# flysnowtiger/GRL

Measured on AMD Instinct MI355X. Metric: clip-features/sec, higher is better.
Workload: dtype f32; 1 GPU; GRL eval clip features (ResNet-50 s1 trunk + GCE + TRL + Siamese attention -> 6144-d), BASELINE configs[1]; clips_per_gpu=32, seq_len=4, frame=256x128, parallelism=replicas x1 (no collective), math=f32

## Files before the change

grl_amd/csrc/gemm_f32.hip:

```cpp
#include <type_traits>
#include <hip/hip_runtime.h>
#include <stdint.h>
#include <stdio.h>
#include <stdlib.h>
#include "../../include/grl_hip.h"
#include "common.h"

namespace {

constexpr int BK = 32;
#ifndef GRL_GEMM_KO
#define GRL_GEMM_KO 0
#endif
constexpr int SEG_STAGES = 16;
#ifndef GRL_GEMM_RING3
#define GRL_GEMM_RING3 1
#endif
#ifndef GRL_GEMM_PIPE
#define GRL_GEMM_PIPE 1
#endif

#ifndef GRL_GEMM_EV_OCC3
#define GRL_GEMM_EV_OCC3 1
#endif

typedef __attribute__((address_space(3))) char* lds_cptr_t;
#pragma clang diagnostic push
#pragma clang diagnostic ignored "-Winline-asm"
__device__ __forceinline__ void dma16_hidden(const char* sbase, uint32_t voff, uint32_t lds) {
    asm volatile("s_mov_b32 m0, %2\n\ts_nop 0\n\tglobal_load_lds_dwordx4 %0, %1" ::"v"(voff), "s"(sbase), "s"(lds) : "memory", "m0");
}
__device__ __forceinline__ void dma16_hidden_v(const char* vaddr, uint32_t lds) {
    asm volatile("s_mov_b32 m0, %1\n\ts_nop 0\n\tglobal_load_lds_dwordx4 %0, off" ::"v"(vaddr), "s"(lds) : "memory", "m0");
}
#pragma clang diagnostic pop

__device__ uint4 g_zero_chunks[8];

struct RowInfo {
    int64_t base;
    int iy0, ix0;
};

constexpr int EV_NONE = 0, EV_AFFINE = 1, EV_SQDIFF = 2;
template <int BM, int BN, bool CONV, int MATH, bool SEG, bool DMA = false, bool SPLITK = false, int EV = EV_NONE>
__global__ __launch_bounds__(256, (GRL_GEMM_EV_OCC3 && EV != EV_NONE && BN == 64) ? 3 : 2) void gemm_f32_kernel(const GrlGemm p_in, const int tiles_n,
                                                                                               const int num_tiles, const int vec_epi_in) {
    static_assert(EV == EV_NONE || (MATH == 0 && BM == 128 && DMA && !SEG && !SPLITK && GRL_GEMM_PIPE), "eval variants: the hand-scheduled fp32 kernels");
    static_assert(EV != EV_SQDIFF || (BN == 128 && !CONV), "SQDIFF: dense, 128 x 128");
    const int vec_epi = EV == EV_NONE ? vec_epi_in : EV == EV_SQDIFF ? (vec_epi_in & 8) | 1 : vec_epi_in & 9;
    GrlGemm p_seg;
    if constexpr (SPLITK) {
        p_seg = p_in;
        const int seg = blockIdx.y, kseg = SEG_STAGES * BK;
        p_seg.a = p_in.a + (int64_t)seg * kseg;
        p_seg.w = p_in.w + (int64_t)seg * kseg;
        p_seg.K = min(kseg, p_in.K - seg * kseg);
        p_seg.y = p_in.splitk_ws + (int64_t)seg * p_in.M * p_in.N;
        p_seg.ldy = p_in.N;
        p_seg.scale = p_seg.shift = p_seg.res = p_seg.gbias = p_seg.rowscale = nullptr;
        p_seg.stats = nullptr;
        p_seg.relu = 0;
    }
    GrlGemm p_ev;
    if constexpr (EV != EV_NONE) {
        p_ev = p_in;
        p_ev.epilogue = EV == EV_SQDIFF ? GRL_EPI_SQDIFF : GRL_EPI_AFFINE;
        p_ev.stats = nullptr;
        p_ev.rowscale = p_ev.rnorm = p_ev.cnorm = nullptr;
        p_ev.bn_z = p_ev.bn_mean = p_ev.bn_invstd = p_ev.bn_mscale = p_ev.bn_mbeta = nullptr;
        p_ev.bn_bits = nullptr;
        p_ev.splitk_ws = nullptr;
        p_ev.kblock = 0;
        p_ev.out_f32 = 0;
        if constexpr (EV == EV_SQDIFF) { p_ev.gbias = nullptr; p_ev.relu = 0; }
    }
    const GrlGemm& p = SPLITK ? p_seg : EV != EV_NONE ? p_ev : p_in;
    constexpr int WTM = BM / 2, WTN = BN / 2;
    constexpr int MT = WTM / 32, NT = WTN / 32;
    constexpr int ESZ = MATH == 2 ? 2 : 4;
    constexpr int EPC = 16 / ESZ;
    constexpr int KST = 8 * EPC;
    auto gp = [](const float* base, int64_t elem_off) {
        return reinterpret_cast<const f32x4*>(reinterpret_cast<const char*>(base) + elem_off * ESZ);
    };
    constexpr int A_ITEMS = BM / 32, B_ITEMS = BN / 32;
    constexpr bool RING = GRL_GEMM_PIPE && GRL_GEMM_RING3 && DMA && MATH == 2 && BM == 128 && BN == 64;
    constexpr int NST = RING ? 3 : 2;
    constexpr bool PIPE = (GRL_GEMM_PIPE && DMA && MATH == 0 && BM == 128) || RING;
    extern __shared__ __attribute__((aligned(16))) float smem[];
    float* As = smem;
    float* Bs = smem + NST * BM * BK;
    constexpr int PL = MATH == 3 ? 2 : 1;
    char* const Ah = reinterpret_cast<char*>(smem);
    char* const Bh = Ah + 2 * PL * BM * 64;

    const int tid = threadIdx.x, lane = tid & 63, wave = PIPE ? __builtin_amdgcn_readfirstlane(tid >> 6) : tid >> 6;
    const int wm = wave >> 1, wn = wave & 1;
    const int ld_row = tid >> 3, ld_chunk = tid & 7;
    const int d_row = lane >> 3, d_chunk = lane & 7;

    RowInfo ai[A_ITEMS];
    int64_t bofs[B_ITEMS];
    const char* dma_a[DMA ? BM / 32 : 1];
    const char* dma_b[DMA ? BN / 32 : 1];
    int dma_iy0[DMA && CONV ? BM / 32 : 1], dma_ix0[DMA && CONV ? BM / 32 : 1];
    const char* cbase[PIPE && CONV ? BM / 32 : 1];
    uint32_t cmask[PIPE && CONV ? BM / 32 : 1];
    uint32_t pv_a[PIPE ? BM / 32 : 1], pv_b[PIPE ? BN / 32 : 1];
    const char *pbase_a = nullptr, *pbase_b = nullptr;
    int m0, n0, tile_m;
    const int tiles_m = num_tiles / tiles_n;
    const int panel_w = (vec_epi & 8) && tiles_n > 8 && (tiles_n & 7) == 0 ? 8 : 0;
    auto setup_tile = [&](int t) {
        int bid = t;
        {
            const int q = num_tiles >> 3, r = num_tiles & 7, xcd = bid & 7;
            bid = (xcd < r ? xcd * (q + 1) : r * (q + 1) + (xcd - r) * q) + (bid >> 3);
        }
        int tile_n;
        if (panel_w > 0) {
            const int per_panel = tiles_m * panel_w;
            const int pn = bid / per_panel, rem = bid - pn * per_panel;
            tile_m = rem / panel_w;
            tile_n = pn * panel_w + (rem - tile_m * panel_w);
        } else {
            tile_m = bid / tiles_n;
            tile_n = bid - tile_m * tiles_n;
        }
        m0 = tile_m * BM;
        n0 = tile_n * BN;
#pragma unroll
        for (int i = 0; i < A_ITEMS; ++i) {
            int m = m0 + ld_row + 32 * i;
            m = m < p.M ? m : p.M - 1;
            if (CONV) {
                const int hw = p.Ho * p.Wo;
                const int img = m / hw, rem = m - img * hw;
                const int oy = rem / p.Wo, ox = rem - oy * p.Wo;
                ai[i].base = (int64_t)img * p.H * p.W * p.C;
                ai[i].iy0 = oy * p.stride - p.pad;
                ai[i].ix0 = ox * p.stride - p.pad;
            } else {
                ai[i].base = (int64_t)m * p.lda;
                ai[i].iy0 = ai[i].ix0 = 0;
            }
        }
#pragma unroll
        for (int i = 0; i < B_ITEMS; ++i) {
            int n = n0 + ld_row + 32 * i;
            n = n < p.N ? n : p.N - 1;
            bofs[i] = (int64_t)n * p.ldw;
        }
        if constexpr (PIPE) {
            pbase_b = reinterpret_cast<const char*>(p.w) + ((int64_t)n0 * p.ldw) * ESZ;
#pragma unroll
            for (int i = 0; i < BN / 32; ++i) {
                const int r = (wave + 4 * i) * 8 + d_row;
                const int n = n0 + r < p.N ? r : p.N - 1 - n0;
                pv_b[i] = (uint32_t)(n * p.ldw * ESZ + ((d_chunk ^ ((r >> 1) & 7)) << 4));
            }
        }
        if constexpr (PIPE && !CONV) {
            pbase_a = reinterpret_cast<const char*>(p.a) + ((int64_t)m0 * p.lda) * ESZ;
#pragma unroll
            for (int i = 0; i < BM / 32; ++i) {
                const int r = (wave + 4 * i) * 8 + d_row;
                const int m = m0 + r < p.M ? r : p.M - 1 - m0;
                pv_a[i] = (uint32_t)(m * p.lda * ESZ + ((d_chunk ^ ((r >> 1) & 7)) << 4));
            }
        } else if constexpr (DMA) {
#pragma unroll
            for (int i = 0; i < BM / 32; ++i) {
                const int r = (wave + 4 * i) * 8 + d_row;
                int m = m0 + r;
                m = m < p.M ? m : p.M - 1;
                if constexpr (CONV) {
                    const int hw = p.Ho * p.Wo;
                    const int img = m / hw, rem = m - img * hw;
                    const int oy = rem / p.Wo, ox = rem - oy * p.Wo;
                    dma_a[i] = reinterpret_cast<const char*>(p.a) + ((int64_t)img * p.H * p.W * p.C) * ESZ + ((d_chunk ^ ((r >> 1) & 7)) << 4);
                    dma_iy0[i] = oy * p.stride - p.pad;
                    dma_ix0[i] = ox * p.stride - p.pad;
                    if constexpr (PIPE) {
                        cbase[i] = dma_a[i] + ((int64_t)(dma_iy0[i] * p.W + dma_ix0[i]) * p.C) * ESZ;
                        uint32_t mk = 0;
                        for (int ky = 0, t = 0; ky < p.kh; ++ky)
                            for (int kx = 0; kx < p.kw; ++kx, ++t)
                                if ((unsigned)(dma_iy0[i] + ky) < (unsigned)p.H && (unsigned)(dma_ix0[i] + kx) < (unsigned)p.W) mk |= 1u << t;
                        cmask[i] = mk;
                    }
                } else {
                    dma_a[i] = reinterpret_cast<const char*>(p.a) + ((int64_t)m * p.lda) * ESZ + ((d_chunk ^ ((r >> 1) & 7)) << 4);
                }
            }
#pragma unroll
            for (int i = 0; i < BN / 32; ++i) {
                const int r = (wave + 4 * i) * 8 + d_row;
                int n = n0 + r;
                n = n < p.N ? n : p.N - 1;
                dma_b[i] = reinterpret_cast<const char*>(p.w) + ((int64_t)n * p.ldw) * ESZ + ((d_chunk ^ ((r >> 1) & 7)) << 4);
            }
        }
    };

    const uint32_t lds_base = (uint32_t)(size_t)((lds_cptr_t) reinterpret_cast<char*>(smem));
    int pky = 0, pkx = 0, pc0 = 0;
    const char* pn_src[PIPE && CONV ? BM / 32 : 1];
    const char* czero = reinterpret_cast<const char*>(g_zero_chunks) + (d_chunk << 4);
    if constexpr (PIPE && CONV) asm volatile("" : "+v"(czero));
    auto conv_tap_reset = [&]() { pky = pkx = pc0 = 0; };
    auto conv_tap_advance = [&]() {
        pc0 += KST;
        if (pc0 >= p.C) {
            pc0 = 0;
            if (++pkx == p.kw) { pkx = 0; ++pky; }
        }
    };
    auto conv_addrs = [&]() {
        if constexpr (PIPE && CONV) {
            const int64_t toff = ((int64_t)(pky * p.W + pkx) * p.C + pc0) * ESZ;
            const uint32_t bit = 1u << (pky * p.kw + pkx);
#pragma unroll
            for (int i = 0; i < BM / 32; ++i)
                pn_src[i] = (cmask[i] & bit) ? cbase[i] + toff : czero;
        }
    };
    auto dma_piece = [&](int buf, int ks, int i) {
        if constexpr (PIPE) {
            const int64_t kb = (int64_t)ks * KST * ESZ;
            if (i < BM / 32) {
                const uint32_t dst = lds_base + (uint32_t)((buf * BM * BK) * 4 + (wave + 4 * i) * 1024);
                if constexpr (CONV) dma16_hidden_v(pn_src[i], dst);
                else dma16_hidden(pbase_a + kb, pv_a[i], dst);
            } else
                dma16_hidden(pbase_b + kb, pv_b[i - BM / 32],
                             lds_base + (uint32_t)((NST * BM * BK + buf * BN * BK) * 4 + (wave + 4 * (i - BM / 32)) * 1024));
        }
    };
    auto dma_stage = [&](int buf, int ks) {
        if constexpr (PIPE) {
            if constexpr (CONV) { conv_tap_reset(); conv_addrs(); }
#pragma unroll
            for (int i = 0; i < BM / 32 + BN / 32; ++i) dma_piece(buf, ks, i);
        } else if constexpr (DMA) {
            if (GRL_GEMM_KO & 8) ks = 0;
            char* const Asb = reinterpret_cast<char*>(As + buf * BM * BK);
            char* const Bsb = reinterpret_cast<char*>(Bs + buf * BN * BK);
            const int64_t kb = (int64_t)ks * KST * ESZ;
            if constexpr (CONV) {
                const int k0 = ks * KST;
                const int tap = k0 / p.C, c0 = k0 - tap * p.C;
                const int ky = tap / p.kw, kx = tap - ky * p.kw;
                const char* const zsrc = reinterpret_cast<const char*>(g_zero_chunks) + (d_chunk << 4);
#pragma unroll
                for (int i = 0; i < BM / 32; ++i) {
                    const int rb = wave + 4 * i;
                    const int iy = dma_iy0[i] + ky, ix = dma_ix0[i] + kx;
                    const bool ok = (unsigned)iy < (unsigned)p.H && (unsigned)ix < (unsigned)p.W;
                    const char* src = ok ? dma_a[i] + ((int64_t)(iy * p.W + ix) * p.C + c0) * ESZ : zsrc;
                    __builtin_amdgcn_global_load_lds((const __attribute__((address_space(1))) void*)src,
                                                     (__attribute__((address_space(3))) void*)(Asb + rb * 1024), 16, 0, 0);
                }
            } else {
#pragma unroll
            for (int i = 0; i < BM / 32; ++i) {
                const int rb = wave + 4 * i;
                __builtin_amdgcn_global_load_lds((const __attribute__((address_space(1))) void*)(dma_a[i] + kb),
                                                 (__attribute__((address_space(3))) void*)(Asb + rb * 1024), 16, 0, 0);
            }
            }
#pragma unroll
            for (int i = 0; i < BN / 32; ++i) {
                const int rb = wave + 4 * i;
                __builtin_amdgcn_global_load_lds((const __attribute__((address_space(1))) void*)(dma_b[i] + kb),
                                                 (__attribute__((address_space(3))) void*)(Bsb + rb * 1024), 16, 0, 0);
            }
        }
    };

    f32x4 areg[A_ITEMS], breg[B_ITEMS];
    auto load_stage = [&](int ks) {
        if constexpr (DMA) return;
        const int k0 = ks * KST;
        if (CONV) {
            const int tap = k0 / p.C, c0 = k0 - tap * p.C;
            const int ky = tap / p.kw, kx = tap - ky * p.kw;
#pragma unroll
            for (int i = 0; i < A_ITEMS; ++i) {
                const int iy = ai[i].iy0 + ky, ix = ai[i].ix0 + kx;
                const bool ok = (unsigned)iy < (unsigned)p.H && (unsigned)ix < (unsigned)p.W;
                const int64_t pix = ok ? (int64_t)iy * p.W + ix : 0;
                f32x4 v = *gp(p.a, ai[i].base + pix * p.C + c0 + ld_chunk * EPC);
#pragma unroll
                for (int e = 0; e < 4; ++e) v[e] = ok ? v[e] : 0.f;
                areg[i] = v;
            }
        } else {
#pragma unroll
            for (int i = 0; i < A_ITEMS; ++i)
                areg[i] = *gp(p.a, ai[i].base + k0 + ld_chunk * EPC);
        }
#pragma unroll
        for (int i = 0; i < B_ITEMS; ++i)
            breg[i] = *gp(p.w, bofs[i] + k0 + ld_chunk * EPC);
    };
    auto split_store = [&](char* plane0, int plane_bytes, int row, const f32x4 v) {
        const int off = row * 64 + (((ld_chunk >> 1) ^ ((row >> 2) & 3)) << 4) + (ld_chunk & 1) * 8;
        bf16x4 hi;
#pragma unroll
        for (int e = 0; e < 4; ++e) hi[e] = (__bf16)v[e];
        *reinterpret_cast<bf16x4*>(plane0 + off) = hi;
        if (MATH == 3) {
            bf16x4 lo;
#pragma unroll
            for (int e = 0; e < 4; ++e) lo[e] = (__bf16)(v[e] - (float)hi[e]);
            *reinterpret_cast<bf16x4*>(plane0 + plane_bytes + off) = lo;
        }
    };
    auto store_stage = [&](int buf) {
        if constexpr (DMA) return;
        if constexpr (MATH == 0 || MATH == 2) {
#pragma unroll
            for (int i = 0; i < A_ITEMS; ++i) {
                const int row = ld_row + 32 * i;
                *reinterpret_cast<f32x4*>(As + buf * BM * BK + row * BK +
                                          ((ld_chunk ^ ((row >> 1) & 7)) << 2)) = areg[i];
            }
#pragma unroll
            for (int i = 0; i < B_ITEMS; ++i) {
                const int row = ld_row + 32 * i;
                *reinterpret_cast<f32x4*>(Bs + buf * BN * BK + row * BK +
                                          ((ld_chunk ^ ((row >> 1) & 7)) << 2)) = breg[i];
            }
        } else {
#pragma unroll
            for (int i = 0; i < A_ITEMS; ++i)
                split_store(Ah + buf * PL * BM * 64, BM * 64, ld_row + 32 * i, areg[i]);
#pragma unroll
            for (int i = 0; i < B_ITEMS; ++i)
                split_store(Bh + buf * PL * BN * 64, BN * 64, ld_row + 32 * i, breg[i]);
        }
    };

    const int nk = p.K / KST;
    const int frow = lane & 31, fhalf = lane >> 5;
    const int col_l = lane & 31;

    int t = blockIdx.x;
    setup_tile(t);
    load_stage(0);
    dma_stage(0, 0);
    for (;;) {
    f32x16 acc[MT][NT], tot[SEG ? MT : 1][SEG ? NT : 1];
#pragma unroll
    for (int i = 0; i < MT; ++i)
#pragma unroll
        for (int j = 0; j < NT; ++j)
#pragma unroll
            for (int r = 0; r < 16; ++r) acc[i][j][r] = 0.f;
    if constexpr (SEG) {
#pragma unroll
        for (int i = 0; i < MT; ++i)
#pragma unroll
            for (int j = 0; j < NT; ++j)
#pragma unroll
                for (int r = 0; r < 16; ++r) tot[i][j][r] = 0.f;
    }

    store_stage(0);
    constexpr int NP_ALL = BM / 32 + BN / 32;
    if constexpr (RING) {
        if (nk > 1) {
            if constexpr (CONV) { conv_tap_advance(); conv_addrs(); }
#pragma unroll
            for (int i = 0; i < NP_ALL; ++i) dma_piece(1, 1, i);
            asm volatile("s_waitcnt vmcnt(%0)" ::"n"(NP_ALL) : "memory");
        } else {
            asm volatile("s_waitcnt vmcnt(0)" ::: "memory");
        }
    } else if constexpr (PIPE) {
        asm volatile("s_waitcnt vmcnt(0)" ::: "memory");
    }
    __syncthreads();

    f32x4 paf[PIPE ? 2 : 1][MT], pbf[PIPE ? 2 : 1][NT];
    auto prd = [&](int set, int buf, int q) {
        if constexpr (PIPE) {
            const float* Ab = As + buf * BM * BK + (wm * WTM) * BK;
            const float* Bb = Bs + buf * BN * BK + (wn * WTN) * BK;
#pragma unroll
            for (int i = 0; i < MT; ++i) {
                const int row = i * 32 + frow;
                paf[set][i] = *reinterpret_cast<const f32x4*>(Ab + row * BK + (((2 * q + fhalf) ^ ((row >> 1) & 7)) << 2));
            }
#pragma unroll
            for (int j = 0; j < NT; ++j) {
                const int row = j * 32 + frow;
                pbf[set][j] = *reinterpret_cast<const f32x4*>(Bb + row * BK + (((2 * q + fhalf) ^ ((row >> 1) & 7)) << 2));
            }
        }
    };
    if constexpr (PIPE) prd(0, 0, 0);

    int rbuf = 0;
    for (int ks = 0; ks < nk; ++ks) {
        const int buf = RING ? rbuf : (ks & 1);
        if constexpr (!PIPE)
            if (!(GRL_GEMM_KO & 1) && ks + 1 < nk) { load_stage(ks + 1); dma_stage(buf ^ 1, ks + 1); }
        if constexpr (RING) {
            const int b1 = buf == 2 ? 0 : buf + 1;
            const int b2 = b1 == 2 ? 0 : b1 + 1;
            const bool more = ks + 1 < nk, more2 = ks + 2 < nk;
            constexpr int NA = BM / 32, NB = BN / 32;
#pragma unroll
            for (int q = 0; q < 4; ++q) {
                if (q < 3) {
                    prd((q + 1) & 1, buf, q + 1);
                } else {
                    if (more2) asm volatile("s_waitcnt vmcnt(%0)" ::"n"(NA + NB) : "memory");
                    else asm volatile("s_waitcnt vmcnt(0)" ::: "memory");
                    __syncthreads();
                    if (more) prd(0, b1, 0);
                }
                __builtin_amdgcn_sched_barrier(0);
#pragma unroll
                for (int i = 0; i < MT; ++i)
#pragma unroll
                    for (int j = 0; j < NT; ++j)
                        acc[i][j] = __builtin_amdgcn_mfma_f32_32x32x16_bf16(__builtin_bit_cast(bf16x8, paf[q & 1][i]),
                                                                            __builtin_bit_cast(bf16x8, pbf[q & 1][j]), acc[i][j], 0, 0, 0);
                if (more2 && q < 2) {
                    const int first = CONV ? (q == 0 ? NA : 0) : (q == 0 ? 0 : (NA + NB) / 2);
                    const int cnt = CONV ? (q == 0 ? NB : NA) : (NA + NB) / 2;
                    __builtin_amdgcn_sched_barrier(0);
#pragma unroll
                    for (int k = 0; k < (CONV ? (NA > NB ? NA : NB) : (NA + NB) / 2); ++k)
                        if (k < cnt) dma_piece(b2, ks + 2, first + k);
                    __builtin_amdgcn_sched_barrier(0);
                    if (CONV && q == 0) { conv_tap_advance(); conv_addrs(); }
                }
                __builtin_amdgcn_sched_barrier(0);
            }
            rbuf = b1;
        } else if constexpr (PIPE) {
            const bool more = ks + 1 < nk;
#pragma unroll
            for (int q = 0; q < 4; ++q) {
                if (q < 3) {
                    prd((q + 1) & 1, buf, q + 1);
                } else {
                    asm volatile("s_waitcnt vmcnt(0)" ::: "memory");
                    __syncthreads();
                    if (more) prd(0, buf ^ 1, 0);
                }
                __builtin_amdgcn_sched_barrier(0);
#pragma unroll
                for (int s = 0; s < 4; ++s) {
#pragma unroll
                    for (int i = 0; i < MT; ++i)
#pragma unroll
                        for (int j = 0; j < NT; ++j)
                            acc[i][j] = __builtin_amdgcn_mfma_f32_32x32x2f32(paf[q & 1][i][s], pbf[q & 1][j][s], acc[i][j], 0, 0, 0);
                    constexpr int NA = BM / 32, NB = BN / 32;
                    const int first = CONV ? (q == 0 ? NA + 2 * s : q == 1 ? 2 * s : -1) : (q == 0 ? 2 * s : -1);
                    const int last = CONV ? (q == 0 ? NA + NB : NA) : NA + NB;
                    if (more && first >= 0 && first < last) {
                        __builtin_amdgcn_sched_barrier(0);
                        dma_piece(buf ^ 1, ks + 1, first);
                        dma_piece(buf ^ 1, ks + 1, first + 1);
                        __builtin_amdgcn_sched_barrier(0);
                    }
                    if (CONV && q == 0 && s == 1 && more) { conv_tap_advance(); conv_addrs(); }
// ... 65 lines not shown
                    const int row = i * 32 + frow;
                    af[i] = *reinterpret_cast<const f32x4*>(
                        Ab + row * BK + (((2 * q + fhalf) ^ ((row >> 1) & 7)) << 2));
                }
#pragma unroll
                for (int j = 0; j < NT; ++j) {
                    const int row = j * 32 + frow;
                    bf[j] = *reinterpret_cast<const f32x4*>(
                        Bb + row * BK + (((2 * q + fhalf) ^ ((row >> 1) & 7)) << 2));
                }
#pragma unroll
                for (int s = 0; s < 4; ++s)
#pragma unroll
                    for (int i = 0; i < MT; ++i)
#pragma unroll
                        for (int j = 0; j < NT; ++j)
                            acc[i][j] = __builtin_amdgcn_mfma_f32_32x32x2f32(af[i][s], bf[j][s],
                                                                             acc[i][j], 0, 0, 0);
            }
            }
        } else {
            const char* Ab = Ah + buf * PL * BM * 64 + (wm * WTM) * 64;
            const char* Bb = Bh + buf * PL * BN * 64 + (wn * WTN) * 64;
#pragma unroll
            for (int s = 0; s < 2; ++s) {
                bf16x8 ah[MT], al[MT], bh[NT], bl[NT];
#pragma unroll
                for (int i = 0; i < MT; ++i) {
                    const int row = i * 32 + frow;
                    const int off = row * 64 + (((2 * s + fhalf) ^ ((row >> 2) & 3)) << 4);
                    ah[i] = *reinterpret_cast<const bf16x8*>(Ab + off);
                    if (MATH == 3) al[i] = *reinterpret_cast<const bf16x8*>(Ab + BM * 64 + off);
                }
#pragma unroll
                for (int j = 0; j < NT; ++j) {
                    const int row = j * 32 + frow;
                    const int off = row * 64 + (((2 * s + fhalf) ^ ((row >> 2) & 3)) << 4);
                    bh[j] = *reinterpret_cast<const bf16x8*>(Bb + off);
                    if (MATH == 3) bl[j] = *reinterpret_cast<const bf16x8*>(Bb + BN * 64 + off);
                }
#pragma unroll
                for (int i = 0; i < MT; ++i)
#pragma unroll
                    for (int j = 0; j < NT; ++j) {
                        if (MATH == 3) {
                            acc[i][j] = __builtin_amdgcn_mfma_f32_32x32x16_bf16(al[i], bh[j], acc[i][j], 0, 0, 0);
                            acc[i][j] = __builtin_amdgcn_mfma_f32_32x32x16_bf16(ah[i], bl[j], acc[i][j], 0, 0, 0);
                        }
                        acc[i][j] = __builtin_amdgcn_mfma_f32_32x32x16_bf16(ah[i], bh[j], acc[i][j], 0, 0, 0);
                    }
            }
        }
        if constexpr (SEG) {
            if (((ks + 1) & (SEG_STAGES - 1)) == 0 && ks + 1 < nk) {
#pragma unroll
                for (int i = 0; i < MT; ++i)
#pragma unroll
                    for (int j = 0; j < NT; ++j) {
                        tot[i][j] += acc[i][j];
#pragma unroll
                        for (int r = 0; r < 16; ++r) acc[i][j][r] = 0.f;
                    }
            }
        }
        if constexpr (!PIPE) {
            if (!(GRL_GEMM_KO & 1) && ks + 1 < nk) store_stage(buf ^ 1);
            if (!(GRL_GEMM_KO & 2)) __syncthreads();
        }
    }
    if constexpr (SEG) {
        if (nk > SEG_STAGES) {
#pragma unroll
            for (int i = 0; i < MT; ++i)
#pragma unroll
                for (int j = 0; j < NT; ++j) acc[i][j] += tot[i][j];
        }
    }

    const int cur_m0 = m0, cur_n0 = n0, cur_tile_m = tile_m;
    const int next_t = t + (int)gridDim.x;
    if (next_t < num_tiles) {
        setup_tile(next_t);
        load_stage(0);
    }

    auto epilogue = [&](const int m0, const int n0, const int tile_m) {
    if (vec_epi & 1) {
        float* Cs = smem;
        if constexpr (!SEG) {
            const bool bnz = p.bn_z != nullptr && p.stats != nullptr;
            const bool fast = p.epilogue == GRL_EPI_AFFINE && !p.rowscale && !p.gbias && (bnz || (!p.stats && !p.bn_z)) &&
                              m0 + BM <= p.M && n0 + BN <= p.N && (MATH != 2 || (!p.out_f32 && p.N % 8 == 0));
            if (fast) {
                auto park = [&]() {
#pragma unroll
                    for (int i = 0; i < MT; ++i)
#pragma unroll
                        for (int j = 0; j < NT; ++j)
#pragma unroll
                            for (int r = 0; r < 16; ++r)
                                Cs[(wm * WTM + i * 32 + (r & 3) + 8 * (r >> 2) + 4 * fhalf) * BN + wn * WTN + j * 32 + col_l] = acc[i][j][r];
                };
                float relu_floor;
            {
                const uint32_t floor_bits = p.relu ? 0u : 0x7fc00000u;
                asm("v_mov_b32 %0, %1" : "=v"(relu_floor) : "s"(floor_bits));
            }
                const bool relu = p.relu != 0;
                auto run = [&](auto has_res_, auto bnz_) {
                    constexpr bool HAS_RES = decltype(has_res_)::value;
                    constexpr bool BNZ = decltype(bnz_)::value;
                    if constexpr (MATH == 2) {
                        constexpr int LPR8 = WTN / 8, RPI8 = 64 / LPR8, NIT = WTM / RPI8, CH = (BM == 128 && BN == 128) ? 2 : (NIT < 4 ? NIT : 4);
                        const int lrow = lane / LPR8, lcol = (lane % LPR8) * 8;
                        const int n = n0 + wn * WTN + lcol;
                        f32x4 sc[2], sh[2];
#pragma unroll
                        for (int u = 0; u < 2; ++u) {
                            sc[u] = p.scale ? *reinterpret_cast<const f32x4*>(p.scale + n + 4 * u) : f32x4{1.f, 1.f, 1.f, 1.f};
                            sh[u] = p.shift ? *reinterpret_cast<const f32x4*>(p.shift + n + 4 * u) : f32x4{0.f, 0.f, 0.f, 0.f};
                        }
                        const __bf16* const r16 = reinterpret_cast<const __bf16*>(p.res);
                        __bf16* const y16 = reinterpret_cast<__bf16*>(p.y);
                        const __bf16* const z16 = reinterpret_cast<const __bf16*>(p.bn_z);
                        const bool use_bits = BNZ && p.bn_bits != nullptr;
                        const bool use_ms = BNZ && !use_bits && p.bn_mscale != nullptr;
                        const uint8_t* const bbyte = use_bits ? p.bn_bits : reinterpret_cast<const uint8_t*>(p.bn_z);
                        f32x4 bmu[2], bis[2], bms[2], bmb[2];
#pragma unroll
                        for (int u = 0; u < 2; ++u) {
                            bmu[u] = bis[u] = bms[u] = bmb[u] = f32x4{0.f, 0.f, 0.f, 0.f};
                            if constexpr (BNZ) {
                                bmu[u] = *reinterpret_cast<const f32x4*>(p.bn_mean + n + 4 * u);
                                bis[u] = *reinterpret_cast<const f32x4*>(p.bn_invstd + n + 4 * u);
                                if (use_ms) {
                                    bms[u] = *reinterpret_cast<const f32x4*>(p.bn_mscale + n + 4 * u);
                                    if (p.bn_mbeta) bmb[u] = *reinterpret_cast<const f32x4*>(p.bn_mbeta + n + 4 * u);
                                }
                            }
                        }
                        f32x4 ssum8[2] = {{0.f, 0.f, 0.f, 0.f}, {0.f, 0.f, 0.f, 0.f}}, ssq8[2] = {{0.f, 0.f, 0.f, 0.f}, {0.f, 0.f, 0.f, 0.f}};
                        bf16x8 r8[2][CH], z8[2][BNZ ? CH : 1];
                        uint32_t bb[2][BNZ ? CH : 1];
                        auto request = [&](int c) {
#pragma unroll
                            for (int k = 0; k < CH; ++k) {
                                const int m = m0 + wm * WTM + (c * CH + k) * RPI8 + lrow;
                                if constexpr (HAS_RES) r8[c & 1][k] = *reinterpret_cast<const bf16x8*>(r16 + (int64_t)m * p.ldres + n);
                                if constexpr (BNZ) {
                                    z8[c & 1][k] = *reinterpret_cast<const bf16x8*>(z16 + (int64_t)m * p.N + n);
                                    bb[c & 1][k] = bbyte[((int64_t)m * p.N + n) >> 3];
                                }
                            }
                        };
                        if constexpr (HAS_RES || BNZ) request(0);
                        park();
#pragma unroll
                        for (int c = 0; c < NIT / CH; ++c) {
                            if constexpr (HAS_RES || BNZ) { if (c + 1 < NIT / CH) request(c + 1); }
#pragma unroll
                            for (int k = 0; k < CH; ++k) {
                                const int row = wm * WTM + (c * CH + k) * RPI8 + lrow;
                                const int m = m0 + row;
                                f32x8 o32;
#pragma unroll
                                for (int u = 0; u < 2; ++u) {
// ... 2 lines not shown
                                    f32x4 tv;
#pragma unroll
                                    for (int e = 0; e < 4; ++e) {
                                        float t = v[e];
                                        if constexpr (HAS_RES) t = t + (float)r8[c & 1][k][4 * u + e];
                                        else t = t + 0.f;
                                        tv[e] = __builtin_fmaxf(t, relu_floor);
                                    }
                                    if constexpr (BNZ) {
                                        f32x4 zc;
#pragma unroll
                                        for (int e = 0; e < 4; ++e) zc[e] = (float)z8[c & 1][k][4 * u + e] - bmu[u][e];
                                        const uint32_t mk = use_bits ? (bb[c & 1][k] >> (4 * u)) : 0xfu;
                                        const f32x4 tm = zc * bms[u] + bmb[u];
#pragma unroll
                                        for (int e = 0; e < 4; ++e) tv[e] = ((((mk >> e) & 1u) != 0) & (!use_ms | (tm[e] > 0.f))) ? tv[e] : 0.f;
                                        ssum8[u] += tv; ssq8[u] += tv * (zc * bis[u]);
                                    }
#pragma unroll
                                    for (int e = 0; e < 4; ++e) o32[4 * u + e] = tv[e];
                                }
                                *reinterpret_cast<bf16x8*>(y16 + (int64_t)m * p.ldy + n) = __builtin_convertvector(o32, bf16x8);
                            }
                        }
                        if constexpr (BNZ) {
#pragma unroll
                            for (int o2 = LPR8; o2 < 64; o2 <<= 1) {
#pragma unroll
                                for (int u = 0; u < 2; ++u)
#pragma unroll
                                    for (int e = 0; e < 4; ++e) {
                                        ssum8[u][e] += __shfl_xor(ssum8[u][e], o2);
                                        ssq8[u][e] += __shfl_xor(ssq8[u][e], o2);
                                    }
                            }
                            __syncthreads();
                            float* red = smem;
                            if (lrow == 0) {
#pragma unroll
                                for (int u = 0; u < 2; ++u) {
                                    *reinterpret_cast<f32x4*>(red + (wm * 2 + 0) * BN + wn * WTN + lcol + 4 * u) = ssum8[u];
                                    *reinterpret_cast<f32x4*>(red + (wm * 2 + 1) * BN + wn * WTN + lcol + 4 * u) = ssq8[u];
                                }
                            }
                            __syncthreads();
                            for (int c = tid; c < BN; c += 256) {
                                const int nn = n0 + c;
                                p.stats[((int64_t)tile_m * 2 + 0) * p.N + nn] = red[0 * BN + c] + red[2 * BN + c];
                                p.stats[((int64_t)tile_m * 2 + 1) * p.N + nn] = red[1 * BN + c] + red[3 * BN + c];
                            }
                        }
                    } else {
                        constexpr int LPR = WTN / 4, RPI = 64 / LPR, NIT = WTM / RPI, CH = (BM == 128 && BN == 128) ? 2 : (NIT < 4 ? NIT : 4);
                        const int lrow = lane / LPR, lcol = (lane % LPR) * 4;
                        const int n = n0 + wn * WTN + lcol;
                        const f32x4 sc = p.scale ? *reinterpret_cast<const f32x4*>(p.scale + n) : f32x4{1.f, 1.f, 1.f, 1.f};
                        const f32x4 sh = p.shift ? *reinterpret_cast<const f32x4*>(p.shift + n) : f32x4{0.f, 0.f, 0.f, 0.f};
                        f32x4 bmu = sh, bis = sh, bms = f32x4{0.f, 0.f, 0.f, 0.f}, bmb = bms;
                        const bool use_bits = BNZ && p.bn_bits != nullptr;
                        if constexpr (BNZ) {
                            bmu = *reinterpret_cast<const f32x4*>(p.bn_mean + n);
                            bis = *reinterpret_cast<const f32x4*>(p.bn_invstd + n);
                            if (!use_bits && p.bn_mscale) {
                                bms = *reinterpret_cast<const f32x4*>(p.bn_mscale + n);
                                bmb = p.bn_mbeta ? *reinterpret_cast<const f32x4*>(p.bn_mbeta + n) : f32x4{0.f, 0.f, 0.f, 0.f};
                            }
                        }
                        const uint8_t* const bbyte = use_bits ? p.bn_bits : reinterpret_cast<const uint8_t*>(p.bn_z);
                        const bool use_ms = BNZ && !use_bits && p.bn_mscale != nullptr;
                        f32x4 ssum = {0.f, 0.f, 0.f, 0.f}, ssq = {0.f, 0.f, 0.f, 0.f};
                        f32x4 rr[2][CH], zz[2][BNZ ? CH : 1];
                        uint32_t bb[2][BNZ ? CH : 1];
                        auto request = [&](int c) {
#pragma unroll
                            for (int k = 0; k < CH; ++k) {
                                const int m = m0 + wm * WTM + (c * CH + k) * RPI + lrow;
                                if constexpr (HAS_RES) rr[c & 1][k] = *reinterpret_cast<const f32x4*>(p.res + (int64_t)m * p.ldres + n);
                                if constexpr (BNZ) {
                                    zz[c & 1][k] = *reinterpret_cast<const f32x4*>(p.bn_z + (int64_t)m * p.N + n);
                                    bb[c & 1][k] = bbyte[((int64_t)m * p.N + n) >> 2];
                                }
                            }
                        };
                        if constexpr (HAS_RES || BNZ) request(0);
                        park();
#pragma unroll
                        for (int c = 0; c < NIT / CH; ++c) {
                            if constexpr (HAS_RES || BNZ) { if (c + 1 < NIT / CH) request(c + 1); }
#pragma unroll
                            for (int k = 0; k < CH; ++k) {
                                const int row = wm * WTM + (c * CH + k) * RPI + lrow;
                                const int m = m0 + row;
                                f32x4 v = *reinterpret_cast<const f32x4*>(Cs + row * BN + wn * WTN + lcol);
                                v = v * sc + sh;
                                if constexpr (HAS_RES) v += rr[c & 1][k];
#pragma unroll
                                for (int e = 0; e < 4; ++e) v[e] = relu ? (v[e] > 0.f ? v[e] : 0.f) : v[e];
                                if constexpr (BNZ) {
                                    const f32x4 zc = zz[c & 1][k] - bmu;
                                    const uint32_t mk = use_bits ? bb[c & 1][k] : 0xfu;
                                    const f32x4 t = zc * bms + bmb;
#pragma unroll
                                    for (int e = 0; e < 4; ++e) v[e] = ((((mk >> e) & 1u) != 0) & (!use_ms | (t[e] > 0.f))) ? v[e] : 0.f;
                                    ssum += v; ssq += v * (zc * bis);
                                }
                                *reinterpret_cast<f32x4*>(p.y + (int64_t)m * p.ldy + n) = v;
                            }
                        }
                        if constexpr (BNZ) {
#pragma unroll
                            for (int o = LPR; o < 64; o <<= 1) {
#pragma unroll
                                for (int e = 0; e < 4; ++e) { ssum[e] += __shfl_xor(ssum[e], o); ssq[e] += __shfl_xor(ssq[e], o); }
                            }
                            __syncthreads();
                            float* red = smem;
                            if (lrow == 0) {
                                *reinterpret_cast<f32x4*>(red + (wm * 2 + 0) * BN + wn * WTN + lcol) = ssum;
                                *reinterpret_cast<f32x4*>(red + (wm * 2 + 1) * BN + wn * WTN + lcol) = ssq;
                            }
                            __syncthreads();
                            for (int c = tid; c < BN; c += 256) {
                                const int nn = n0 + c;
                                p.stats[((int64_t)tile_m * 2 + 0) * p.N + nn] = red[0 * BN + c] + red[2 * BN + c];
                                p.stats[((int64_t)tile_m * 2 + 1) * p.N + nn] = red[1 * BN + c] + red[3 * BN + c];
                            }
                        }
                    }
                };
                if (bnz) {
                    if (p.res) run(std::true_type{}, std::true_type{});
                    else run(std::false_type{}, std::true_type{});
                } else if (p.res) run(std::true_type{}, std::false_type{});
                else run(std::false_type{}, std::false_type{});
                return;
            }
        }
        constexpr int EPI_ROWS = WTM / (64 / (WTN / 4));
        constexpr bool RES_PREFETCH = MATH != 2 && !SEG && !(BM == 128 && BN == 128);
        constexpr int EPI_UNROLL = RES_PREFETCH ? EPI_ROWS : 4;
        f32x4 rpre[RES_PREFETCH ? EPI_ROWS : 1];
        f32x4 zpre[RES_PREFETCH ? EPI_ROWS : 1];
        uint32_t bpre[RES_PREFETCH ? EPI_ROWS : 1];
        if constexpr (RES_PREFETCH) {
            constexpr int LPRp = WTN / 4, RPIp = 64 / LPRp;
            const int np = n0 + wn * WTN + (lane % LPRp) * 4;
            if (p.res && p.epilogue == GRL_EPI_AFFINE) {
#pragma unroll
                for (int it = 0; it < EPI_ROWS; ++it) {
                    const int m = m0 + wm * WTM + it * RPIp + lane / LPRp;
                    if (m < p.M && np < p.N) rpre[it] = *reinterpret_cast<const f32x4*>(p.res + (int64_t)m * p.ldres + np);
                }
            }
            if (p.bn_z && p.epilogue == GRL_EPI_AFFINE) {
#pragma unroll
                for (int it = 0; it < EPI_ROWS; ++it) {
                    const int m = m0 + wm * WTM + it * RPIp + lane / LPRp;
                    if (m < p.M && np < p.N) {
                        zpre[it] = *reinterpret_cast<const f32x4*>(p.bn_z + (int64_t)m * p.N + np);
                        if (p.bn_bits) bpre[it] = p.bn_bits[((int64_t)m * p.N + np) >> 2];
                    }
                }
            }
        }
#pragma unroll
        for (int i = 0; i < MT; ++i)
#pragma unroll
            for (int j = 0; j < NT; ++j)
#pragma unroll
                for (int r = 0; r < 16; ++r)
                    Cs[(wm * WTM + i * 32 + (r & 3) + 8 * (r >> 2) + 4 * fhalf) * BN + wn * WTN +
                       j * 32 + col_l] = acc[i][j][r];
        if constexpr (MATH == 2) {
            if (p.N % 8 == 0 && !p.out_f32 && !p.rowscale) {
                constexpr int LPR8 = WTN / 8, RPI8 = 64 / LPR8;
                const int lrow = lane / LPR8, lcol = (lane % LPR8) * 8;
// ... 289 lines not shown
                    if (nn < p.N) {
                        p.stats[((int64_t)tile_m * 2 + 0) * p.N + nn] = red[0 * BN + c] + red[2 * BN + c];
                        p.stats[((int64_t)tile_m * 2 + 1) * p.N + nn] = red[1 * BN + c] + red[3 * BN + c];
                    }
                }
            }
        }
        return;
    }
    float csum[NT], csq[NT];
#pragma unroll
    for (int j = 0; j < NT; ++j) csum[j] = csq[j] = 0.f;

#pragma unroll
    for (int j = 0; j < NT; ++j) {
        const int n = n0 + wn * WTN + j * 32 + col_l;
        const bool n_ok = n < p.N;
        const int nn = n_ok ? n : p.N - 1;
        const float sc = p.scale ? p.scale[nn] : 1.f;
        const float sh = p.shift ? p.shift[nn] : 0.f;
        const float cn = (p.epilogue == GRL_EPI_EUCLID) ? p.cnorm[nn] : 0.f;
#pragma unroll
        for (int i = 0; i < MT; ++i) {
#pragma unroll
            for (int r = 0; r < 16; ++r) {
                const int m = m0 + wm * WTM + i * 32 + (r & 3) + 8 * (r >> 2) + 4 * fhalf;
                if (m >= p.M) continue;
                float v = acc[i][j][r];
                if (p.epilogue == GRL_EPI_AFFINE) {
                    if (p.rowscale) v *= p.rowscale[m];
                    if (p.gbias) v += p.gbias[(int64_t)(m / p.rows_per_group) * p.N + nn];
                    if (p.stats) { csum[j] += v; csq[j] += v * v; }
                    v = v * sc + sh;
                    if (p.res && n_ok) v += p.res[(int64_t)m * p.ldres + n];
                    if (p.relu) v = v > 0.f ? v : 0.f;
                } else if (p.epilogue == GRL_EPI_NEGDOT) {
                    v = -v;
                } else {
                    v = p.rnorm[m] + cn - 2.f * v;
                    v = sqrtf(v > 1e-12f ? v : 1e-12f);
                }
                if (n_ok) p.y[(int64_t)m * p.ldy + n] = v;
            }
        }
    }

    if (p.stats) {
        __syncthreads();
        float* red = smem;
#pragma unroll
        for (int j = 0; j < NT; ++j) {
            float s = csum[j] + __shfl_xor(csum[j], 32);
            float q2 = csq[j] + __shfl_xor(csq[j], 32);
            if (fhalf == 0) {
                const int c = wn * WTN + j * 32 + col_l;
                red[(wm * 2 + 0) * BN + c] = s;
                red[(wm * 2 + 1) * BN + c] = q2;
            }
        }
        __syncthreads();
        for (int c = tid; c < BN; c += 256) {
            const int n = n0 + c;
            if (n < p.N) {
                p.stats[((int64_t)tile_m * 2 + 0) * p.N + n] = red[0 * BN + c] + red[2 * BN + c];
                p.stats[((int64_t)tile_m * 2 + 1) * p.N + n] = red[1 * BN + c] + red[3 * BN + c];
            }
        }
    }
    };
    if constexpr ((GRL_GEMM_KO & 4) != 0) {
        float s = 0.f;
#pragma unroll
        for (int i = 0; i < MT; ++i)
#pragma unroll
            for (int j = 0; j < NT; ++j)
#pragma unroll
                for (int r = 0; r < 16; ++r) s += acc[i][j][r];
        if (s == 1.2345e-30f) p.y[0] = s;
    } else {
        epilogue(cur_m0, cur_n0, cur_tile_m);
    }
    if (next_t >= num_tiles) break;
    t = next_t;
    __syncthreads();
    dma_stage(0, 0);
    }
}

__global__ void splitk_finish_kernel(const GrlGemm p, const int nseg) {
    const int64_t total = (int64_t)p.M * p.N, plane = total;
    for (int64_t i = blockIdx.x * (int64_t)blockDim.x + threadIdx.x; i < total; i += (int64_t)gridDim.x * blockDim.x) {
        const int m = (int)(i / p.N), n = (int)(i - (int64_t)m * p.N);
        float tot = 0.f;
        for (int sgm = 0; sgm + 1 < nseg; ++sgm) tot += p.splitk_ws[(int64_t)sgm * plane + i];
        float v = p.splitk_ws[(int64_t)(nseg - 1) * plane + i];
        v += tot;
        const float sc = p.scale ? p.scale[n] : 1.f, sh = p.shift ? p.shift[n] : 0.f;
        v = v * sc + sh;
        if (p.res) v += p.res[(int64_t)m * p.ldres + n];
        if (p.relu) v = v > 0.f ? v : 0.f;
        p.y[(int64_t)m * p.ldy + n] = v;
    }
}

int64_t splitk_floats(const GrlGemm& d) {
    if (d.math != GRL_MATH_F32 || !d.kblock || d.conv || d.stats || d.gbias || d.rowscale || d.epilogue != GRL_EPI_AFFINE)
        return 0;
    if (d.M > 256 || d.K <= SEG_STAGES * BK) return 0;
    const int64_t tiles = (int64_t)((d.M + 63) / 64) * ((d.N + 63) / 64);
    if (tiles > 128) return 0;
    const int nseg = (d.K + SEG_STAGES * BK - 1) / (SEG_STAGES * BK);
    return (int64_t)nseg * d.M * d.N;
}

struct TileChoice { int bm, bn, smode = 0; };
int g_force_tile = 0;

TileChoice legacy_tile(const GrlGemm& d) {
    if (d.epilogue == GRL_EPI_SQDIFF) return {128, 128};
    static const TileChoice forced = [] {
        TileChoice f{0, 0, 0};
        if (const char* e = getenv("GRL_GEMM_TILE")) {
            int bm = 0, bn = 0;
            if (sscanf(e, "%dx%d", &bm, &bn) == 2 && (bm == 128 || bm == 64) && (bn == 128 || bn == 64) &&
                !(bm == 64 && bn == 128))
                f = {bm, bn};
        }
        return f;
    }();
    if (g_force_tile) return {g_force_tile >> 16, g_force_tile & 0xffff};
    if (forced.bm) return forced;
    auto tiles = [&](int bm, int bn) {
        return (int64_t)((d.M + bm - 1) / bm) * ((d.N + bn - 1) / bn);
    };
    if (d.N <= 64) return tiles(128, 64) >= 512 ? TileChoice{128, 64} : TileChoice{64, 64};
    static const bool wide_on = [] { const char* e = getenv("GRL_GEMM_WIDE"); return !e || atoi(e) != 0; }();
    static const bool wide3_on = [] { const char* e = getenv("GRL_GEMM_WIDE3"); return !e || atoi(e) != 0; }();
    static const int bnz_narrow_k = [] { const char* e = getenv("GRL_GEMM_BNZ_NARROW"); return e ? atoi(e) : 512; }();
    const bool bnz_narrow = d.bn_z && d.math == GRL_MATH_F32 && d.K <= bnz_narrow_k;
    if (wide_on && !bnz_narrow && (!d.stats || d.bn_z) && (d.math == GRL_MATH_F32 || (wide3_on && d.math != GRL_MATH_BF16S)) && d.N >= 128 &&
        tiles(128, 128) >= (d.conv ? 448 : 256) && !(d.res && d.K <= (d.stats ? 128 : 512)))
        return {128, 128};
    if (d.K <= 128 && d.res && !d.stats && d.math == GRL_MATH_F32 && d.N >= 128 && tiles(128, 128) >= 448) return {128, 128};
    if (d.K <= 128) return {64, 64};
    if (d.K <= 512) return tiles(128, 64) >= ((d.stats || d.conv) ? 448 : 256) ? TileChoice{128, 64} : TileChoice{64, 64};
    if (tiles(128, 128) >= 448) return {128, 128};
    if (tiles(128, 64) >= (d.conv ? 448 : 256)) return {128, 64};
    return {64, 64};
}

bool vec_epilogue_ok(const GrlGemm& d) {
    auto al16 = [](const void* q) { return ((uintptr_t)q & 15) == 0; };
    return d.N % 4 == 0 && d.ldy % 4 == 0 && al16(d.y) && (!d.res || (d.ldres % 4 == 0 && al16(d.res))) && al16(d.scale) &&
           al16(d.shift) && al16(d.gbias) && al16(d.cnorm);
}

TileChoice choose_tile(const GrlGemm& d) {
    TileChoice t = legacy_tile(d);
    const char* const ws_env = getenv("GRL_GEMM_WIDE_STATS");
    const bool wide_stats = !ws_env || atoi(ws_env) != 0;
    static const bool forced_env = getenv("GRL_GEMM_TILE") != nullptr;
    const bool forced = forced_env || g_force_tile != 0;
    if (!wide_stats || forced || !d.stats || d.bn_z || d.math == GRL_MATH_BF16S || d.epilogue != GRL_EPI_AFFINE || d.N < 128 ||
        !vec_epilogue_ok(d) || ((uintptr_t)d.stats & 15) != 0)
        return t;
    const int64_t tiles128 = (int64_t)((d.M + 127) / 128) * ((d.N + 127) / 128);
    if (tiles128 < 448) return t;
    if (t.bm == 64 && t.bn == 64) return {128, 128, 1};
    if (t.bm == 128 && t.bn == 64) return {128, 128, 2};
    return t;
}

int resident_workgroups(const void* kernel, size_t lds) {
    if (lds > 65536) (void)hipFuncSetAttribute(kernel, hipFuncAttributeMaxDynamicSharedMemorySize, (int)lds);
    static const int forced_grid = [] {
        const char* e = getenv("GRL_GEMM_GRID");
        return e ? atoi(e) : -1;
    }();
    if (forced_grid >= 0) return forced_grid > 0 ? (forced_grid + 7) / 8 * 8 : 0x7fffffff;
    int dev = 0, cus = 256, occ = 2;
    if (hipGetDevice(&dev) == hipSuccess) {
        hipDeviceProp_t prop;
        if (hipGetDeviceProperties(&prop, dev) == hipSuccess && prop.multiProcessorCount > 0)
            cus = prop.multiProcessorCount;
    }
    if (hipOccupancyMaxActiveBlocksPerMultiprocessor(&occ, kernel, 256, lds) != hipSuccess || occ < 1) occ = 2;
    (void)hipGetLastError();
    return (cus * occ + 7) / 8 * 8;
}

template <auto KERNEL>
void launch_kernel(const GrlGemm& d, hipStream_t s, size_t lds, int tiles_n, int num_tiles, int vec_epi) {
    static int slots_of[16] = {0};
    int dev = 0;
    (void)hipGetDevice(&dev);
    int& cached = slots_of[dev & 15];
    if (cached == 0) cached = resident_workgroups((const void*)KERNEL, lds);
    const int slots = cached;
    hipLaunchKernelGGL(KERNEL, dim3(num_tiles < slots ? num_tiles : slots), dim3(256), lds, s, d, tiles_n, num_tiles,
                       vec_epi);
}

int eval_variant(const GrlGemm& d, int bm, int bn, int vec_epi) {
    if (d.math != GRL_MATH_F32 || bm != 128 || d.stats || d.bn_z || d.rowscale || d.kblock) return EV_NONE;
    if (d.epilogue == GRL_EPI_SQDIFF ? !(bn == 128 && (vec_epi & 1)) : d.epilogue != GRL_EPI_AFFINE) return EV_NONE;
    const char* const e = getenv("GRL_GEMM_EVAL_VARIANT");
    if (e && atoi(e) == 0) return EV_NONE;
    return d.epilogue == GRL_EPI_SQDIFF ? EV_SQDIFF : EV_AFFINE;
}

void debug_name(int bm, int bn, const GrlGemm& d, int math, bool seg, bool dma, int ev) {
    if (!getenv("GRL_DEBUG_SYNC")) return;
    fprintf(stderr, "[grl] gemm_f32_kernel<%d,%d,conv=%d,math=%d,seg=%d,dma=%d> variant=%s\n", bm, bn, d.conv ? 1 : 0, math, seg ? 1 : 0,
            dma ? 1 : 0, ev == EV_AFFINE ? "eval" : ev == EV_SQDIFF ? "eval-sqdiff" : "generic");
}

template <int BM, int BN, int MATH>
int launch_math(const GrlGemm& d, hipStream_t s, int smode) {
    const int tiles_m = (d.M + BM - 1) / BM, tiles_n = (d.N + BN - 1) / BN;
    const int num_tiles = tiles_m * tiles_n;
    constexpr int NST = (GRL_GEMM_PIPE && GRL_GEMM_RING3 && MATH == 2 && BM == 128 && BN == 64) ? 3 : 2;
    constexpr size_t stage_bytes = (MATH == 0 || MATH == 2) ? (size_t)NST * (BM + BN) * BK * sizeof(float)
                                                            : (size_t)2 * (MATH == 3 ? 2 : 1) * (BM + BN) * 64;
    constexpr size_t c_bytes = (size_t)BM * BN * sizeof(float);
    constexpr size_t lds = stage_bytes > c_bytes ? stage_bytes : c_bytes;
    static const bool panel_on = [] { const char* e = getenv("GRL_GEMM_PANEL"); return !e || atoi(e) != 0; }();
    const int vec_epi = (vec_epilogue_ok(d) ? 1 | (smode << 1) : 0) | (panel_on ? 8 : 0);
    if (MATH == 2 && !(vec_epi & 1))
        return grl_fail(GRL_EINVAL, "gemm bf16s: y/res/scale/shift/gbias must be 16-byte aligned");
    if (MATH == 2 && d.bn_z && (d.M % BM || d.N % BN))
        return grl_fail(GRL_EINVAL, "gemm bf16s: bn_z on a %d x %d tile needs M, N multiples of the tile", BM, BN);
    constexpr bool CAN_SEG = MATH == 0;
    const bool seg = CAN_SEG && d.kblock && d.K > SEG_STAGES * BK;
    static const bool dma_conv_on = [] { const char* e = getenv("GRL_GEMM_DMA_CONV"); return !e || atoi(e) != 0; }();
    constexpr bool CAN_EV = GRL_GEMM_PIPE && MATH == 0 && BM == 128;
    const int ev = CAN_EV ? eval_variant(d, BM, BN, vec_epi) : EV_NONE;
    if (d.conv) {
        constexpr bool CAN_DMA_CONV = (MATH == 0 || MATH == 2) && BM == 128;
        const bool dma = CAN_DMA_CONV && dma_conv_on && d.ldw < (1 << 22) && d.kh * d.kw <= 32;
        debug_name(BM, BN, d, MATH, seg, dma, dma ? ev : EV_NONE);
        if constexpr (CAN_EV) {
            if (dma && ev == EV_AFFINE) {
                launch_kernel<gemm_f32_kernel<BM, BN, true, MATH, false, true, false, EV_AFFINE>>(d, s, lds, tiles_n, num_tiles, vec_epi);
                return grl_check_launch("grl_conv_gemm_f32");
            }
        }
        if (dma) {
            if (seg) launch_kernel<gemm_f32_kernel<BM, BN, true, MATH, CAN_SEG, CAN_DMA_CONV>>(d, s, lds, tiles_n, num_tiles, vec_epi);
            else launch_kernel<gemm_f32_kernel<BM, BN, true, MATH, false, CAN_DMA_CONV>>(d, s, lds, tiles_n, num_tiles, vec_epi);
        } else if (seg) launch_kernel<gemm_f32_kernel<BM, BN, true, MATH, CAN_SEG>>(d, s, lds, tiles_n, num_tiles, vec_epi);
        else launch_kernel<gemm_f32_kernel<BM, BN, true, MATH, false>>(d, s, lds, tiles_n, num_tiles, vec_epi);
    } else {
        static const bool dma_on = [] { const char* e = getenv("GRL_GEMM_DMA"); return !e || atoi(e) != 0; }();
        constexpr bool CAN_DMA = (MATH == 0 || MATH == 2) && BM == 128;
        static const int dma_mink = [] { const char* e = getenv("GRL_GEMM_DMA_MINK"); return e ? atoi(e) : 256; }();
        const bool dma = CAN_DMA && dma_on && d.K >= dma_mink && d.lda < (1 << 22) && d.ldw < (1 << 22);
        debug_name(BM, BN, d, MATH, seg, dma, dma ? ev : EV_NONE);
        if constexpr (CAN_EV) {
            if (dma && ev == EV_AFFINE) {
                launch_kernel<gemm_f32_kernel<BM, BN, false, MATH, false, true, false, EV_AFFINE>>(d, s, lds, tiles_n, num_tiles, vec_epi);
                return grl_check_launch("grl_conv_gemm_f32");
            }
            if constexpr (BN == 128) {
                if (dma && ev == EV_SQDIFF) {
                    launch_kernel<gemm_f32_kernel<BM, BN, false, MATH, false, true, false, EV_SQDIFF>>(d, s, lds, tiles_n, num_tiles, vec_epi);
                    return grl_check_launch("grl_conv_gemm_f32");
                }
            }
        }
        if (dma) {
            if (seg) launch_kernel<gemm_f32_kernel<BM, BN, false, MATH, CAN_SEG, CAN_DMA>>(d, s, lds, tiles_n, num_tiles, vec_epi);
            else launch_kernel<gemm_f32_kernel<BM, BN, false, MATH, false, CAN_DMA>>(d, s, lds, tiles_n, num_tiles, vec_epi);
        } else if (seg) launch_kernel<gemm_f32_kernel<BM, BN, false, MATH, CAN_SEG>>(d, s, lds, tiles_n, num_tiles, vec_epi);
        else launch_kernel<gemm_f32_kernel<BM, BN, false, MATH, false>>(d, s, lds, tiles_n, num_tiles, vec_epi);
    }
    return grl_check_launch("grl_conv_gemm_f32");
}

template <int BM, int BN>
int launch(const GrlGemm& d, hipStream_t s, int smode = 0) {
    if (d.math == GRL_MATH_BF16S) return launch_math<BM, BN, 2>(d, s, 0);
    if (d.math == GRL_MATH_BF16X3) return launch_math<BM, BN, 3>(d, s, smode);
    if (d.math == GRL_MATH_BF16) return launch_math<BM, BN, 1>(d, s, smode);
    return launch_math<BM, BN, 0>(d, s, smode);
}

int validate(const GrlGemm& d) {
    if (!d.a || !d.w || !d.y) return grl_fail(GRL_EINVAL, "gemm: null operand");
    if (d.M <= 0 || d.N <= 0 || d.K <= 0) return grl_fail(GRL_EINVAL, "gemm: empty shape");
    if (d.K % BK) return grl_fail(GRL_EINVAL, "gemm: K must be a multiple of 32");
    if (d.ldw % 4 || ((uintptr_t)d.w & 15) || ((uintptr_t)d.a & 15))
        return grl_fail(GRL_EINVAL, "gemm: operands must be 16-byte aligned with ld % 4 == 0");
    if (d.conv) {
        if (d.C % BK) return grl_fail(GRL_EINVAL, "conv: C must be a multiple of 32");
        if (d.K != d.kh * d.kw * d.C) return grl_fail(GRL_EINVAL, "conv: K != kh*kw*C");
        if (d.M % (d.Ho * d.Wo)) return grl_fail(GRL_EINVAL, "conv: M must be nimg*Ho*Wo");
    } else if (d.lda % 4) {
// ... 98 lines not shown
```

Before: 2240 clip-features/sec.

## Overlap next tile's first-stage DMA with the affine eval epilogue

For the eval affine GEMM variant, the LDS layout changes so that stage buffer 0 holds both A and B for one stage. Stage buffer 1 can then hold half of the C tile at a time. The next tile's first-stage DMA is issued before the epilogue runs, and accumulators are parked in two halves instead of all at once, so global loads overlap epilogue work. This removes the barrier and stage-0 load that used to follow the epilogue in the persistent tile loop. The cost is a more complex LDS layout and an extra parking pass per half; the path only applies to full interior tiles without gbias.

```diff
diff --git a/grl_amd/csrc/gemm_f32.hip b/grl_amd/csrc/gemm_f32.hip
--- a/grl_amd/csrc/gemm_f32.hip
+++ b/grl_amd/csrc/gemm_f32.hip
@@ -22,6 +22,9 @@
 
 #ifndef GRL_GEMM_EV_OCC3
 #define GRL_GEMM_EV_OCC3 1
+#endif
+#ifndef GRL_GEMM_EPI_EARLY
+#define GRL_GEMM_EPI_EARLY 1
 #endif
 
 typedef __attribute__((address_space(3))) char* lds_cptr_t;
@@ -88,9 +91,14 @@
     constexpr bool RING = GRL_GEMM_PIPE && GRL_GEMM_RING3 && DMA && MATH == 2 && BM == 128 && BN == 64;
     constexpr int NST = RING ? 3 : 2;
     constexpr bool PIPE = (GRL_GEMM_PIPE && DMA && MATH == 0 && BM == 128) || RING;
+    constexpr bool EARLY = GRL_GEMM_EPI_EARLY != 0 && EV == EV_AFFINE;
+    constexpr int A_BUF = EARLY ? (BM + BN) * BK : BM * BK;
+    constexpr int B_BUF = EARLY ? (BM + BN) * BK : BN * BK;
+    constexpr int B_OFF = EARLY ? BM * BK : NST * BM * BK;
+    static_assert(!EARLY || (NST == 2 && MT == 2 && 64 * BN <= (BM + BN) * BK), "EARLY: half a C tile fits the second stage buffer");
     extern __shared__ __attribute__((aligned(16))) float smem[];
     float* As = smem;
-    float* Bs = smem + NST * BM * BK;
+    float* Bs = smem + B_OFF;
     constexpr int PL = MATH == 3 ? 2 : 1;
     char* const Ah = reinterpret_cast<char*>(smem);
     char* const Bh = Ah + 2 * PL * BM * 64;
@@ -230,12 +238,12 @@
         if constexpr (PIPE) {
             const int64_t kb = (int64_t)ks * KST * ESZ;
             if (i < BM / 32) {
-                const uint32_t dst = lds_base + (uint32_t)((buf * BM * BK) * 4 + (wave + 4 * i) * 1024);
+                const uint32_t dst = lds_base + (uint32_t)((buf * A_BUF) * 4 + (wave + 4 * i) * 1024);
                 if constexpr (CONV) dma16_hidden_v(pn_src[i], dst);
                 else dma16_hidden(pbase_a + kb, pv_a[i], dst);
             } else
                 dma16_hidden(pbase_b + kb, pv_b[i - BM / 32],
-                             lds_base + (uint32_t)((NST * BM * BK + buf * BN * BK) * 4 + (wave + 4 * (i - BM / 32)) * 1024));
+                             lds_base + (uint32_t)((B_OFF + buf * B_BUF) * 4 + (wave + 4 * (i - BM / 32)) * 1024));
         }
     };
     auto dma_stage = [&](int buf, int ks) {
@@ -387,8 +395,8 @@
     f32x4 paf[PIPE ? 2 : 1][MT], pbf[PIPE ? 2 : 1][NT];
     auto prd = [&](int set, int buf, int q) {
         if constexpr (PIPE) {
-            const float* Ab = As + buf * BM * BK + (wm * WTM) * BK;
-            const float* Bb = Bs + buf * BN * BK + (wn * WTN) * BK;
+            const float* Ab = As + buf * A_BUF + (wm * WTM) * BK;
+            const float* Bb = Bs + buf * B_BUF + (wn * WTN) * BK;
 #pragma unroll
             for (int i = 0; i < MT; ++i) {
                 const int row = i * 32 + frow;
@@ -620,6 +628,12 @@
     if (next_t < num_tiles) {
         setup_tile(next_t);
         load_stage(0);
+    }
+    bool early = false;
+    if constexpr (EARLY) {
+        __builtin_amdgcn_s_waitcnt(0x0f70);
+        early = next_t < num_tiles && (vec_epi & 1) && !p.gbias && cur_m0 + BM <= p.M && cur_n0 + BN <= p.N;
+        if (early) dma_stage(0, 0);
     }
 
     auto epilogue = [&](const int m0, const int n0, const int tile_m) {
@@ -788,16 +802,28 @@
                                 }
                             }
                         };
+                        constexpr int HCH = NIT / CH / 2;
+                        static_assert(!EARLY || (HCH >= 1 && HCH * CH * RPI == 32), "EARLY: a half pass is whole chunks");
+                        float* const Ch = smem + (BM + BN) * BK + wave * (32 * WTN);
+                        auto park_half = [&](int h) {
+#pragma unroll
+                            for (int j = 0; j < NT; ++j)
+#pragma unroll
+                                for (int r = 0; r < 16; ++r)
+                                    Ch[((r & 3) + 8 * (r >> 2) + 4 * fhalf) * WTN + j * 32 + col_l] = acc[h][j][r];
+                        };
                         if constexpr (HAS_RES || BNZ) request(0);
-                        park();
+                        if constexpr (!EARLY) park();
 #pragma unroll
                         for (int c = 0; c < NIT / CH; ++c) {
+                            if constexpr (EARLY) { if (c % HCH == 0) park_half(c / HCH); }
                             if constexpr (HAS_RES || BNZ) { if (c + 1 < NIT / CH) request(c + 1); }
 #pragma unroll
                             for (int k = 0; k < CH; ++k) {
                                 const int row = wm * WTM + (c * CH + k) * RPI + lrow;
                                 const int m = m0 + row;
-                                f32x4 v = *reinterpret_cast<const f32x4*>(Cs + row * BN + wn * WTN + lcol);
+                                f32x4 v = EARLY ? *reinterpret_cast<const f32x4*>(Ch + (((c % HCH) * CH + k) * RPI + lrow) * WTN + lcol)
+                                                : *reinterpret_cast<const f32x4*>(Cs + row * BN + wn * WTN + lcol);
                                 v = v * sc + sh;
                                 if constexpr (HAS_RES) v += rr[c & 1][k];
 #pragma unroll
@@ -1253,6 +1279,9 @@
     }
     if (next_t >= num_tiles) break;
     t = next_t;
+    if constexpr (EARLY) {
+        if (early) continue;
+    }
     __syncthreads();
     dma_stage(0, 0);
     }
@@ -1382,8 +1411,8 @@
 
 void debug_name(int bm, int bn, const GrlGemm& d, int math, bool seg, bool dma, int ev) {
     if (!getenv("GRL_DEBUG_SYNC")) return;
-    fprintf(stderr, "[grl] gemm_f32_kernel<%d,%d,conv=%d,math=%d,seg=%d,dma=%d> variant=%s\n", bm, bn, d.conv ? 1 : 0, math, seg ? 1 : 0,
-            dma ? 1 : 0, ev == EV_AFFINE ? "eval" : ev == EV_SQDIFF ? "eval-sqdiff" : "generic");
+    fprintf(stderr, "[grl] gemm_f32_kernel<%d,%d,conv=%d,math=%d,seg=%d,dma=%d> variant=%s epi_early=%d\n", bm, bn, d.conv ? 1 : 0, math, seg ? 1 : 0,
+            dma ? 1 : 0, ev == EV_AFFINE ? "eval" : ev == EV_SQDIFF ? "eval-sqdiff" : "generic", ev == EV_AFFINE && GRL_GEMM_EPI_EARLY ? 1 : 0);
 }
 
 template <int BM, int BN, int MATH>
```

Result: no change. 2235 clip-features/sec (-0.2%).
